# nrclaudio/spVIPES

Measured on AMD Instinct MI355X. Metric: cells/sec/training-step (2-group PoE VAE), higher is better.
Workload: dtype bf16

## Files before the change

include/spvipes_hip.h:

```cpp
#ifndef SPVIPES_HIP_H
#define SPVIPES_HIP_H

#include <stdint.h>

#ifdef __cplusplus
extern "C" {
#endif

#define SPV_OK 0
#define SPV_ERR_ARG (-1)
#define SPV_ERR_LAUNCH (-2)
#define SPV_ERR_UNSUPPORTED (-3)

#define SPV_COUNT_F32 0
#define SPV_COUNT_U16 1

#define SPV_NB_CMAX 64
#define SPV_DEC_KP 16
#define SPV_DEC_KS 32
#define SPV_DEC_KP_WIDE 32
#define SPV_DEC_KS_WIDE 64
#define SPV_DEC_CELLS_PER_WG 128

int spv_version(void);
// ... 109 lines not shown
int spv_dec_heads_wgrad(const uint16_t* tP, const uint16_t* tS, int32_t a_tiles, const uint16_t* Aps, int32_t G, int32_t Bp,
                        int32_t splits, float* slabP, float* slabS, void* stream);

int spv_dec_logits(const uint16_t* Am_hi, const uint16_t* Am_lo, const uint16_t* Wm_hi, const uint16_t* Wm_lo,
                   int32_t K, int32_t Bp, int32_t Gp, int32_t nsplit, void* out, int32_t out_f32, void* stream);

typedef struct spv_dec_params {
  const void* X; int64_t ldx; const int32_t* rows; int32_t col_off; int32_t count_is_u16;
  int32_t B, G, Bp, Gp;
  const void* logits; int32_t n_gene_tiles; int32_t logits_f32;
  const uint16_t* Wps_hi; const uint16_t* Wps_lo;
  const uint16_t* Aps_hi; const uint16_t* Aps_lo;
  const void* gene_tab;
  const void* cnt_tab;
  const float* a_p; const float* a_s; const float* lse_p; const float* lse_s;
  const float* w_row;
  int32_t gene_splits; int32_t genes_per_split;
  float* part_max_p; float* part_sum_p; float* part_max_s; float* part_sum_s;
  float* rec_part; float* tp_part; float* ts_part;
  float* dtheta_part;
  void* dL; void* tP; void* tS; int32_t grads_f32;
  int32_t nb_splits; int32_t nb_genes_per_split;
  int32_t nb_cell_tiles;
  int32_t kslots;
} spv_dec_params;

int spv_dec_tables(const float* px_r, int32_t G, int32_t Gp, void* gene_tab, void* cnt_tab, void* stream);

int spv_dec_lse(const spv_dec_params* p, const float* library, void* stream);

int spv_dec_nb_fwd(const spv_dec_params* p, int32_t train, void* stream);

typedef struct spv_dec_group {
  spv_dec_params p;
  const float* library;
  const float* px_r;
  const uint16_t* Am_hi; const uint16_t* Am_lo; const uint16_t* Wm_hi; const uint16_t* Wm_lo; int32_t K, nsplit;
  const float* Tp; const float* Ts; float* dz_part; float* dw_part;
} spv_dec_group;
int spv_dec_tables_grouped(const spv_dec_group* groups, int32_t n_groups, void* stream);
int spv_dec_logits_grouped(const spv_dec_group* groups, int32_t n_groups, void* stream);
int spv_dec_lse_grouped(const spv_dec_group* groups, int32_t n_groups, void* stream);
int spv_dec_nb_fwd_grouped(const spv_dec_group* groups, int32_t n_groups, int32_t train, void* stream);
int spv_dec_heads_bwd_grouped(const spv_dec_group* groups, int32_t n_groups, void* stream);

int spv_dec_materialize(const spv_dec_params* p, float* scale_private, float* scale_shared, float* rate_private, float* rate_shared,
// ... 259 lines not shown
```

spvipes_amd/_abi.py:

```python
from __future__ import annotations

import ctypes as C
import os
from typing import NamedTuple, Optional

import torch

_HERE = os.path.dirname(os.path.abspath(__file__))
LIB_PATH = os.path.join(_HERE, "_lib", "libspvipes_hip.so")

SPV_COUNT_F32, SPV_COUNT_U16 = 0, 1
NB_CMAX, DEC_KP, DEC_KS, DEC_CELLS_PER_WG = 64, 16, 32, 128
DEC_KPS = DEC_KP + DEC_KS


class DecSlots(NamedTuple):
    kslots: int
    KP: int
    KS: int
    KPS: int


DEC_NARROW = DecSlots(0, DEC_KP, DEC_KS, DEC_KPS)
DEC_WIDE = DecSlots(1, 32, 64, 96)


class SpvCounts(C.Structure):
    _fields_ = [("X", C.c_void_p), ("ld", C.c_int64), ("rows", C.c_void_p), ("col_off", C.c_int32), ("dtype", C.c_int32)]


class SpvDecParams(C.Structure):
    _fields_ = [
        ("X", C.c_void_p), ("ldx", C.c_int64), ("rows", C.c_void_p), ("col_off", C.c_int32), ("count_is_u16", C.c_int32),
        ("B", C.c_int32), ("G", C.c_int32), ("Bp", C.c_int32), ("Gp", C.c_int32),
        ("logits", C.c_void_p), ("n_gene_tiles", C.c_int32), ("logits_f32", C.c_int32),
        ("Wps_hi", C.c_void_p), ("Wps_lo", C.c_void_p), ("Aps_hi", C.c_void_p), ("Aps_lo", C.c_void_p),
        ("gene_tab", C.c_void_p), ("cnt_tab", C.c_void_p),
        ("a_p", C.c_void_p), ("a_s", C.c_void_p), ("lse_p", C.c_void_p), ("lse_s", C.c_void_p), ("w_row", C.c_void_p),
        ("gene_splits", C.c_int32), ("genes_per_split", C.c_int32),
        ("part_max_p", C.c_void_p), ("part_sum_p", C.c_void_p), ("part_max_s", C.c_void_p), ("part_sum_s", C.c_void_p),
        ("rec_part", C.c_void_p), ("tp_part", C.c_void_p), ("ts_part", C.c_void_p), ("dtheta_part", C.c_void_p),
        ("dL", C.c_void_p), ("tP", C.c_void_p), ("tS", C.c_void_p), ("grads_f32", C.c_int32),
        ("nb_splits", C.c_int32), ("nb_genes_per_split", C.c_int32), ("nb_cell_tiles", C.c_int32),
        ("kslots", C.c_int32),
    ]


class SpvReduceProb(C.Structure):
    _fields_ = [("src", C.c_void_p), ("slab_stride", C.c_int64), ("ld_src", C.c_int64), ("nslabs", C.c_int32), ("col_off", C.c_int32),
                ("rows", C.c_int32), ("cols", C.c_int32), ("dst", C.c_void_p), ("ld_dst", C.c_int64), ("accumulate", C.c_int32),
                ("pad_", C.c_int32), ("alpha", C.c_void_p), ("exp_scale", C.c_void_p)]


SPV_MAXR = 16


class SpvReduceBatch(C.Structure):
    _fields_ = [("p", SpvReduceProb * SPV_MAXR), ("nprob", C.c_int32)]


SPV_MAXP = 8
POE_LMAX = 1024
BN_ROWS = 32


class SpvLinearProb(C.Structure):
# ... 346 lines not shown
```

spvipes_amd/csrc/spv_abi.hip:

```cpp
#include "../../include/spvipes_hip.h"
#include "spv_common.h"
#include "spv_gemm.h"
#include "spv_fc1.h"
#include "spv_dec_gemm.h"
#include "spv_decoder.h"
#include "spv_dec_expected.h"
#include "spv_de.h"
#include "spv_de_median.h"
#include "spv_small.h"
#include "spv_poe_n.h"

#include <cstdio>
#include <cstdlib>
#include <cstring>

using namespace spv;

static thread_local char g_err[512] = "";
static int fail(int code, const char* fmt, const char* what = "") {
  snprintf(g_err, sizeof(g_err), fmt, what);
  return code;
}
static int launch_status(const char* what) {
  hipError_t e = hipGetLastError();
// ... 456 lines not shown
    return fail(SPV_ERR_ARG, "spv_dec_heads_wgrad: operands must be 16-byte aligned%s");
  static bool raised = false;
  if (!raised) { (void)hipFuncSetAttribute(reinterpret_cast<const void*>(dec_heads_wgrad_dma_kernel), hipFuncAttributeMaxDynamicSharedMemorySize, DH_LDS_BYTES); raised = true; }
  const int mtiles = (G + DH_BM - 1) / DH_BM, ktiles = Bp / DH_BK;
  const int k_per_split = (ktiles + splits - 1) / splits * DH_BK;
  hipLaunchKernelGGL(dec_heads_wgrad_dma_kernel, dim3(mtiles * splits), dim3(512), DH_LDS_BYTES, (hipStream_t)stream, (const bf16_t*)tP, (const bf16_t*)tS, a_tiles,
                     (const bf16_t*)Aps, G, Bp, k_per_split, splits, slabP, slabS);
  return launch_status("spv_dec_heads_wgrad");
}

static int to_dec(const spv_dec_params* q, DecParams& p) {
  if (!q) return fail(SPV_ERR_ARG, "decoder: null params%s");
  p.X = q->X; p.ldx = q->ldx; p.rows = q->rows; p.col_off = q->col_off; p.count_is_u16 = q->count_is_u16;
  p.B = q->B; p.G = q->G; p.Bp = q->Bp; p.Gp = q->Gp;
  p.logits = q->logits; p.n_gene_tiles = q->n_gene_tiles; p.logits_f32 = q->logits_f32;
  p.Wps_hi = q->Wps_hi; p.Wps_lo = q->Wps_lo; p.Aps_hi = q->Aps_hi; p.Aps_lo = q->Aps_lo;
  p.gene_tab = (const float4*)q->gene_tab; p.cnt_tab = (const float2*)q->cnt_tab;
  p.a_p = q->a_p; p.a_s = q->a_s; p.lse_p = q->lse_p; p.lse_s = q->lse_s; p.w_row = q->w_row;
  p.gene_splits = q->gene_splits; p.genes_per_split = q->genes_per_split;
  p.part_max_p = q->part_max_p; p.part_sum_p = q->part_sum_p; p.part_max_s = q->part_max_s; p.part_sum_s = q->part_sum_s;
  p.rec_part = q->rec_part; p.tp_part = q->tp_part; p.ts_part = q->ts_part; p.dtheta_part = q->dtheta_part;
  p.dL = q->dL; p.tP = q->tP; p.tS = q->tS; p.grads_f32 = q->grads_f32;
  p.nb_splits = q->nb_splits; p.nb_genes_per_split = q->nb_genes_per_split; p.nb_cell_tiles = q->nb_cell_tiles > 0 ? q->nb_cell_tiles : 1;
  if (p.B <= 0 || p.G <= 0 || p.Bp < p.B || p.Gp < p.G || (p.Bp % DEC_CELLS_PER_WG) || (p.Gp % 32))
    return fail(SPV_ERR_ARG, "decoder: Bp must be a multiple of 128 and Gp of 32%s");
  if ((long)p.Bp * p.Gp * (p.grads_f32 ? 2 : 1) >= (1L << 30) || p.Gp >= (1 << 24))
    return fail(SPV_ERR_ARG, "decoder: Bp * Gp must stay below 2^30 elements (and Gp below 2^24)%s");
  if (p.gene_splits <= 0 || (p.genes_per_split % 32) || (long)p.gene_splits * p.genes_per_split < p.G)
    return fail(SPV_ERR_ARG, "decoder: gene splits must be multiples of 32 covering G%s");
  if (!p.Wps_hi || !p.Wps_lo || !p.Aps_hi || !p.Aps_lo) return fail(SPV_ERR_ARG, "decoder: missing packed regressor operands%s");
  if (q->kslots != 0 && q->kslots != 1) return fail(SPV_ERR_ARG, "decoder: kslots must be 0 (16 / 32 K slots) or 1 (32 / 64)%s");
  return SPV_OK;
}
static inline int dec_kw(const spv_dec_params* q) { return q->kslots ? 2 : 1; }

extern "C" int spv_dec_tables(const float* px_r, int32_t G, int32_t Gp, void* gene_tab, void* cnt_tab, void* stream) {
  if (!px_r || !gene_tab || !cnt_tab || G <= 0 || Gp < G) return fail(SPV_ERR_ARG, "spv_dec_tables: bad arguments%s");
  hipLaunchKernelGGL(nb_tables_kernel, dim3((Gp + 255) / 256, NB_CMAX), dim3(256), 0, (hipStream_t)stream, px_r, G, Gp,
                     (float4*)gene_tab, (float2*)cnt_tab);
  return launch_status("spv_dec_tables");
}

extern "C" int spv_dec_tables_grouped(const spv_dec_group* g, int32_t n, void* stream) {
  if (!g || n <= 0) return fail(SPV_ERR_ARG, "spv_dec_tables_grouped: bad arguments%s");
  int i = 0;
  for (; i + 1 < n; i += 2) {
// ... 37 lines not shown
  int i = 0;
  for (; i + 1 < n; i += 2) {
    DecParams p0, p1;
    int rc = lse_prepare(&g[i].p, g[i].library, p0);
    if (rc != SPV_OK) return rc;
    rc = lse_prepare(&g[i + 1].p, g[i + 1].library, p1);
    if (rc != SPV_OK) return rc;
    if (dec_kw(&g[i].p) != dec_kw(&g[i + 1].p)) break;
    const int bp = p0.Bp > p1.Bp ? p0.Bp : p1.Bp, gs = p0.gene_splits > p1.gene_splits ? p0.gene_splits : p1.gene_splits;
    if (dec_kw(&g[i].p) == 2) hipLaunchKernelGGL(dec_lse_pair_kernel<2>, dim3(bp / DEC_CELLS_PER_WG, gs, 2), dim3(256), 0, s, p0, p1);
    else hipLaunchKernelGGL(dec_lse_pair_kernel<1>, dim3(bp / DEC_CELLS_PER_WG, gs, 2), dim3(256), 0, s, p0, p1);
    const LseCombArgs c0{p0.part_max_p, p0.part_sum_p, p0.part_max_s, p0.part_sum_s, p0.gene_splits, p0.Bp, p0.B, g[i].library, (float*)p0.lse_p, (float*)p0.lse_s, (float*)p0.a_p, (float*)p0.a_s};
    const LseCombArgs c1{p1.part_max_p, p1.part_sum_p, p1.part_max_s, p1.part_sum_s, p1.gene_splits, p1.Bp, p1.B, g[i + 1].library, (float*)p1.lse_p, (float*)p1.lse_s, (float*)p1.a_p, (float*)p1.a_s};
    hipLaunchKernelGGL(dec_lse_combine_pair_kernel, dim3((bp + 63) / 64, 1, 2), dim3(256), 0, s, c0, c1);
    if (hipGetLastError() != hipSuccess) return launch_status("spv_dec_lse_grouped");
  }
  for (; i < n; ++i) {
    const int rc = spv_dec_lse(&g[i].p, g[i].library, stream);
    if (rc != SPV_OK) return rc;
  }
  return SPV_OK;
}

template <bool TRAIN, typename GT, int CM, int KW>
static void nb_launch_mode(const DecParams& p, hipStream_t s) {
  const int ctiles = (p.Bp + NB_CELLS_PER_WG - 1) / NB_CELLS_PER_WG;
  dim3 grid((ctiles + p.nb_cell_tiles - 1) / p.nb_cell_tiles, p.nb_splits);
  if (p.logits_f32) hipLaunchKernelGGL((dec_nb_kernel<TRAIN, GT, float, CM, KW>), grid, dim3(256), 0, s, p);
  else hipLaunchKernelGGL((dec_nb_kernel<TRAIN, GT, _Float16, CM, KW>), grid, dim3(256), 0, s, p);
}
template <bool TRAIN, typename GT, int KW>
static void nb_launch_kw(const DecParams& p, hipStream_t s) {
  if (!p.count_is_u16) return nb_launch_mode<TRAIN, GT, CNT_F32, KW>(p, s);
  const bool aligned = ((reinterpret_cast<uintptr_t>(p.X) & 7) == 0) && (p.ldx % 4 == 0) && (p.col_off % 4 == 0);
  if (aligned) nb_launch_mode<TRAIN, GT, CNT_U16_ALIGNED, KW>(p, s);
  else nb_launch_mode<TRAIN, GT, CNT_U16_ANY, KW>(p, s);
}
template <bool TRAIN, typename GT>
static void nb_launch(const DecParams& p, int kw, hipStream_t s) {
  if (kw == 2) nb_launch_kw<TRAIN, GT, 2>(p, s);
  else nb_launch_kw<TRAIN, GT, 1>(p, s);
}

static int nb_prepare(const spv_dec_params* q, int32_t train, DecParams& p) {
  int rc = to_dec(q, p);
  if (rc != SPV_OK) return rc;
  if (!p.X || !p.logits || !p.gene_tab || !p.cnt_tab || !p.a_p || !p.a_s || !p.w_row || !p.rec_part)
    return fail(SPV_ERR_ARG, "spv_dec_nb_fwd: null pointer%s");
  if (p.n_gene_tiles != p.Gp / 32) return fail(SPV_ERR_ARG, "spv_dec_nb_fwd: n_gene_tiles must be Gp / 32%s");
  if (p.nb_splits <= 0 || p.nb_genes_per_split <= 0 || (p.nb_genes_per_split % 32) || p.nb_genes_per_split > NB_GSPL_MAX ||
      (long)p.nb_splits * p.nb_genes_per_split < p.G)
    return fail(SPV_ERR_ARG, "spv_dec_nb_fwd: nb_genes_per_split must be a multiple of 32, at most 160, and the splits must cover G%s");
  if (train && (!p.dL || !p.tP || !p.tS || !p.tp_part || !p.ts_part || !p.dtheta_part))
    return fail(SPV_ERR_ARG, "spv_dec_nb_fwd: training outputs missing%s");
  return SPV_OK;
}
extern "C" int spv_dec_nb_fwd(const spv_dec_params* q, int32_t train, void* stream) {
  DecParams p;
  int rc = nb_prepare(q, train, p);
  if (rc != SPV_OK) return rc;
  hipStream_t s = (hipStream_t)stream;
  const int kw = dec_kw(q);
  if (train) {
    if (p.grads_f32) nb_launch<true, split_t>(p, kw, s);
    else nb_launch<true, bf16_t>(p, kw, s);
  } else {
    nb_launch<false, bf16_t>(p, kw, s);
  }
  return launch_status("spv_dec_nb_fwd");
}
static int nb_count_mode(const DecParams& p) {
// ... 9 lines not shown
  else hipLaunchKernelGGL((dec_nb_pair_kernel<TRAIN, GT, _Float16, CM, KW>), grid, dim3(256), 0, s, p0, p1);
}
template <bool TRAIN, typename GT, int KW>
static void nb_launch_pair_kw(const DecParams& p0, const DecParams& p1, int cm, hipStream_t s) {
  if (cm == CNT_F32) nb_launch_pair_mode<TRAIN, GT, CNT_F32, KW>(p0, p1, s);
  else if (cm == CNT_U16_ALIGNED) nb_launch_pair_mode<TRAIN, GT, CNT_U16_ALIGNED, KW>(p0, p1, s);
  else nb_launch_pair_mode<TRAIN, GT, CNT_U16_ANY, KW>(p0, p1, s);
}
template <bool TRAIN, typename GT>
static void nb_launch_pair(const DecParams& p0, const DecParams& p1, int cm, int kw, hipStream_t s) {
  if (kw == 2) nb_launch_pair_kw<TRAIN, GT, 2>(p0, p1, cm, s);
  else nb_launch_pair_kw<TRAIN, GT, 1>(p0, p1, cm, s);
}
extern "C" int spv_dec_nb_fwd_grouped(const spv_dec_group* g, int32_t n, int32_t train, void* stream) {
  if (!g || n <= 0) return fail(SPV_ERR_ARG, "spv_dec_nb_fwd_grouped: bad arguments%s");
  hipStream_t s = (hipStream_t)stream;
  int i = 0;
  for (; i + 1 < n; i += 2) {
    DecParams p0, p1;
    int rc = nb_prepare(&g[i].p, train, p0);
    if (rc != SPV_OK) return rc;
    rc = nb_prepare(&g[i + 1].p, train, p1);
    if (rc != SPV_OK) return rc;
    if (nb_count_mode(p0) != nb_count_mode(p1) || p0.logits_f32 != p1.logits_f32 || p0.grads_f32 != p1.grads_f32 || dec_kw(&g[i].p) != dec_kw(&g[i + 1].p)) break;
    const int cm = nb_count_mode(p0), kw = dec_kw(&g[i].p);
    if (train) {
      if (p0.grads_f32) nb_launch_pair<true, split_t>(p0, p1, cm, kw, s);
      else nb_launch_pair<true, bf16_t>(p0, p1, cm, kw, s);
    } else {
      nb_launch_pair<false, bf16_t>(p0, p1, cm, kw, s);
    }
    if (hipGetLastError() != hipSuccess) return launch_status("spv_dec_nb_fwd_grouped");
  }
  for (; i < n; ++i) {
    const int rc = spv_dec_nb_fwd(&g[i].p, train, stream);
    if (rc != SPV_OK) return rc;
  }
  return SPV_OK;
}

extern "C" int spv_dec_logits(const uint16_t* Am_hi, const uint16_t* Am_lo, const uint16_t* Wm_hi, const uint16_t* Wm_lo,
                              int32_t K, int32_t Bp, int32_t Gp, int32_t nsplit, void* out, int32_t out_f32, void* stream) {
  if (!Am_hi || !Wm_hi || !out) return fail(SPV_ERR_ARG, "spv_dec_logits: null pointer%s");
  if (K <= 0 || (K % 32) || Bp <= 0 || Gp <= 0 || (Bp % 128) || (Gp % 128)) return fail(SPV_ERR_ARG, "spv_dec_logits: bad shape%s");
  if (nsplit != 1 && nsplit != 3) return fail(SPV_ERR_ARG, "spv_dec_logits: nsplit must be 1 or 3%s");
  if (nsplit == 3 && (!Am_lo || !Wm_lo)) return fail(SPV_ERR_ARG, "spv_dec_logits: nsplit=3 needs lo images%s");
// ... 1385 lines not shown
```

spvipes_amd/csrc/spv_decoder.h:

```cpp
#pragma once
#include "spv_common.h"

namespace spv {

constexpr int NB_CMAX = 64;
constexpr int DEC_KP = 16;
constexpr int DEC_KS = 32;
constexpr int DEC_KPS = DEC_KP + DEC_KS;
template <int KW> constexpr int DEC_KP_W = 16 * KW;
template <int KW> constexpr int DEC_KS_W = 32 * KW;
template <int KW> constexpr int DEC_KPS_W = 48 * KW;
constexpr int DEC_CELLS_PER_WG = 128;

struct DecParams {
  const void* X; long ldx; const int* rows; int col_off; int count_is_u16;
  int B, G;
  int Bp, Gp;
  const void* logits; int n_gene_tiles; int logits_f32;
  const bf16_t* Wps_hi; const bf16_t* Wps_lo;
  const bf16_t* Aps_hi; const bf16_t* Aps_lo;
  const float4* gene_tab;
  const float2* cnt_tab;
  const float* a_p; const float* a_s;
  const float* lse_p; const float* lse_s;
  const float* w_row;
  int gene_splits; int genes_per_split;
  float* part_max_p; float* part_sum_p; float* part_max_s; float* part_sum_s;
  float* rec_part; float* tp_part; float* ts_part;
  float* dtheta_part;
  void* dL; void* tP; void* tS; int grads_f32;
  int nb_splits; int nb_genes_per_split;
  int nb_cell_tiles;
};

__device__ __forceinline__ void nb_tables_body(const float* px_r, int G, int Gp, float4* gene_tab, float2* cnt_tab) {
  const int g = blockIdx.x * blockDim.x + threadIdx.x;
  const int c = blockIdx.y;
  if (g >= Gp) return;
  if (g >= G) {
    if (c == 0) gene_tab[g] = make_float4(1.f, 0.f, 1.f, 0.f);
    cnt_tab[(long)c * Gp + g] = make_float2(0.f, 0.f);
    return;
  }
  const float theta = fast_exp(px_r[g]);
  if (c == 0) {
    const float lt = fast_log(theta + SPV_EPS_NB);
    gene_tab[g] = make_float4(theta, lt, fmaf(theta, fast_rcp(theta + SPV_EPS_NB), lt), theta * lt * 1.4426950408889634f);
    cnt_tab[g] = make_float2(0.f, 0.f);
    return;
  }
  const float x = log1p_count((float)c);
  const LgammaDigamma t = lgamma_digamma(theta), xt = lgamma_digamma(x + theta), x1 = lgamma_digamma(x + 1.0f);
  cnt_tab[(long)c * Gp + g] = make_float2(xt.lg - t.lg - x1.lg, xt.dg - t.dg);
}
__global__ void nb_tables_kernel(const float* px_r, int G, int Gp, float4* gene_tab, float2* cnt_tab) { nb_tables_body(px_r, G, Gp, gene_tab, cnt_tab); }
// ... 294 lines not shown

typedef __attribute__((ext_vector_type(4))) float f4acc;
constexpr float NB_LN2 = 0.6931471805599453f, NB_LOG2E = 1.4426950408889634f;
constexpr int NB_GSPL_MAX = 160;
constexpr int NB_WPITCH = 56;
constexpr int NB_CELLS_PER_WG = 64;

#ifndef SPV_NB_ABLATE
#define SPV_NB_ABLATE 0
#endif
#ifdef SPV_NB_STAMPS
__device__ unsigned long long* g_nb_stamps;
#define NB_STAMP(i) do { if (threadIdx.x == 0) { unsigned long long t_; asm volatile("s_memtime %0\n\ts_waitcnt lgkmcnt(0)" : "=s"(t_) :: "memory"); g_nb_stamps[((size_t)blockIdx.y * gridDim.x + blockIdx.x) * 8 + (i)] = t_; } } while (0)
#else
#define NB_STAMP(i) do { } while (0)
#endif
#ifndef SPV_NB_OCC
#define SPV_NB_OCC 3
#endif
constexpr int NB_WPITCH_WIDE = 104;
constexpr int SPV_NB_OCC_WIDE = 2;
template <int KW> constexpr int NB_WPITCH_W = KW == 1 ? NB_WPITCH : NB_WPITCH_WIDE;
template <int KW> constexpr int NB_OCC_W = KW == 1 ? SPV_NB_OCC : SPV_NB_OCC_WIDE;
template <bool TRAIN, typename GT, typename LT, int CM, int KW = 1>
__device__ __forceinline__ void dec_nb_body(const DecParams& p) {
  constexpr int DEC_KP = DEC_KP_W<KW>, DEC_KPS = DEC_KPS_W<KW>, NB_WPITCH = NB_WPITCH_W<KW>;
  constexpr int NSK = DEC_KS_W<KW> / 32;
  __shared__ __attribute__((aligned(16))) bf16_t s_whi[NB_GSPL_MAX * NB_WPITCH], s_wlo[NB_GSPL_MAX * NB_WPITCH];
  __shared__ float4 s_gt[NB_GSPL_MAX];
  __shared__ float s_dth[TRAIN ? 4 : 1][NB_GSPL_MAX];
  const int tid = threadIdx.x, lane = tid & 63, wave = tid >> 6;
  const int c16 = lane & 15, gq = lane >> 4;
  const int split = blockIdx.y;
  const int gbeg = split * p.nb_genes_per_split;
  int gend = gbeg + p.nb_genes_per_split;
  if (gend > p.Gp) gend = p.Gp;
  if (gend > ((p.G + 15) & ~15)) gend = (p.G + 15) & ~15;
  const int ng = gend - gbeg;
  NB_STAMP(0);
  const int nct = p.nb_cell_tiles;
  if (ng <= 0) {
    for (int ct = 0; ct < nct; ++ct) {
      const int cell = (blockIdx.x * nct + ct) * NB_CELLS_PER_WG + tid;
      if (cell < p.Bp) {
        const long o = (long)split * p.Bp + cell;
        p.rec_part[o] = 0.f;
        if constexpr (TRAIN) { p.tp_part[o] = 0.f; p.ts_part[o] = 0.f; }
      }
    }
    return;
  }
  for (int i = tid; i < ng * (DEC_KPS / 8); i += 256) {
    const int row = i / (DEC_KPS / 8), ch = i % (DEC_KPS / 8);
    *reinterpret_cast<u4v*>(s_whi + row * NB_WPITCH + 8 * ch) = *reinterpret_cast<const u4v*>(p.Wps_hi + (long)(gbeg + row) * DEC_KPS + 8 * ch);
    *reinterpret_cast<u4v*>(s_wlo + row * NB_WPITCH + 8 * ch) = *reinterpret_cast<const u4v*>(p.Wps_lo + (long)(gbeg + row) * DEC_KPS + 8 * ch);
  }
  for (int i = tid; i < ng; i += 256) s_gt[i] = p.gene_tab[gbeg + i];
  __syncthreads();
  NB_STAMP(1);
  const int nchunks = ng >> 4;

  for (int ct = 0; ct < nct; ++ct) {
    const int tile16 = (blockIdx.x * nct + ct) * (NB_CELLS_PER_WG / 16) + wave;
    if (tile16 * 16 >= p.Bp) break;
    const int cell = tile16 * 16 + c16;
    const int cell_tile = tile16 >> 1, chh = tile16 & 1;
    const bool cell_ok = cell < p.B;
    const long aoff = (long)cell * DEC_KPS + 8 * gq;
    s8v bp_hi = *reinterpret_cast<const s8v*>(p.Aps_hi + aoff), bp_lo = *reinterpret_cast<const s8v*>(p.Aps_lo + aoff);
    if (DEC_KP == 16 && gq >= 2) {
#pragma unroll
      for (int i = 0; i < 8; ++i) { bp_hi[i] = 0; bp_lo[i] = 0; }
    }
    s8v bs_hi[NSK], bs_lo[NSK];
#pragma unroll
    for (int s = 0; s < NSK; ++s) {
      bs_hi[s] = *reinterpret_cast<const s8v*>(p.Aps_hi + aoff + DEC_KP + 32 * s);
      bs_lo[s] = *reinterpret_cast<const s8v*>(p.Aps_lo + aoff + DEC_KP + 32 * s);
    }
    const float ap2 = p.a_p[cell] * NB_LOG2E, as2 = p.a_s[cell] * NB_LOG2E;
    const float w = p.w_row[cell];
    const long row_of_cell = ((SPV_NB_ABLATE & 16) != 0) ? 0 : (cell_ok ? (p.rows ? (long)p.rows[cell] : (long)cell) : 0);
    float rec = 0.f, tp_sum = 0.f, ts_sum = 0.f;
    const int lane_st = (16 * chh + c16 + 32 * (gq & 1)) * 4 + (gq >> 1) * 256;
    const unsigned tile_row = (unsigned)cell_tile * (unsigned)p.n_gene_tiles;
    const unsigned plane = (unsigned)p.Bp * (unsigned)p.Gp;
    auto tile_off = [&](int g0) { return (tile_row + (unsigned)(g0 >> 5)) * 1024u + (unsigned)(((g0 >> 4) & 1) * 512 + lane_st); };
    auto gather_tab = [&](const float (&c)[4], int g0, float2 (&tab)[4]) {
#pragma unroll
      for (int j = 0; j < 4; ++j) {
        unsigned eo = __umul24((unsigned)(int)__builtin_amdgcn_fmed3f(c[j], 0.f, (float)(NB_CMAX - 1)), (unsigned)p.Gp) + (unsigned)(g0 + 4 * gq + j);
        if constexpr ((SPV_NB_ABLATE & 2) != 0) eo = (unsigned)(g0 + 4 * gq + j);
        tab[j] = *reinterpret_cast<const float2*>(reinterpret_cast<const char*>(p.cnt_tab) + (size_t)(eo * 8u));
      }
    };

    RawCounts<CM> rawA = load_counts4_raw<CM>(p, row_of_cell, gbeg + 4 * gq, cell_ok), rawB = rawA, rawC = rawA;
    float ellA[4];
    float2 tabA[4];
    load4b<LT>(p.logits, tile_off(gbeg), ellA);
    if (nchunks > 1) rawB = load_counts4_raw<CM>(p, row_of_cell, gbeg + 16 + 4 * gq, cell_ok);
    {
      float c0[4];
      decode_counts4<CM>(p, rawA, row_of_cell, gbeg + 4 * gq, cell_ok, c0);
      gather_tab(c0, gbeg, tabA);
    }

    NB_STAMP(2);
    for (int c = 0; c < nchunks; ++c) {
      if (c == 1) NB_STAMP(3);
      const int g0 = gbeg + 16 * c;
      const unsigned toff = tile_off(g0);
      const int wrow = (16 * c + c16) * NB_WPITCH + 8 * gq;
      const s8v wp_hi = *reinterpret_cast<const s8v*>(s_whi + wrow), wp_lo = *reinterpret_cast<const s8v*>(s_wlo + wrow);
      f4acc yp = {0.f, 0.f, 0.f, 0.f}, ys = {0.f, 0.f, 0.f, 0.f};
      yp = __builtin_amdgcn_mfma_f32_16x16x32_bf16(wp_hi, bp_lo, yp, 0, 0, 0);
      yp = __builtin_amdgcn_mfma_f32_16x16x32_bf16(wp_lo, bp_hi, yp, 0, 0, 0);
      yp = __builtin_amdgcn_mfma_f32_16x16x32_bf16(wp_hi, bp_hi, yp, 0, 0, 0);
#pragma unroll
      for (int s = 0; s < NSK; ++s) {
        const s8v ws_hi = *reinterpret_cast<const s8v*>(s_whi + wrow + DEC_KP + 32 * s), ws_lo = *reinterpret_cast<const s8v*>(s_wlo + wrow + DEC_KP + 32 * s);
        ys = __builtin_amdgcn_mfma_f32_16x16x32_bf16(ws_hi, bs_lo[s], ys, 0, 0, 0);
        ys = __builtin_amdgcn_mfma_f32_16x16x32_bf16(ws_lo, bs_hi[s], ys, 0, 0, 0);
        ys = __builtin_amdgcn_mfma_f32_16x16x32_bf16(ws_hi, bs_hi[s], ys, 0, 0, 0);
      }
      const int g1 = gbeg + 16 * min(c + 1, nchunks - 1), g2 = gbeg + 16 * min(c + 2, nchunks - 1);
      float ellB[4];
      float2 tabB[4];
      rawC = load_counts4_raw<CM>(p, row_of_cell, g2 + 4 * gq, cell_ok);
      if constexpr ((SPV_NB_ABLATE & 4) != 0) { ellB[0] = ellA[1]; ellB[1] = ellA[2]; ellB[2] = ellA[3]; ellB[3] = ellA[0]; }
      else load4b<LT>(p.logits, tile_off(g1), ellB);
      {
        float cB[4];
        decode_counts4<CM>(p, rawB, row_of_cell, g1 + 4 * gq, cell_ok, cB);
        gather_tab(cB, g1, tabB);
      }
      float cntA[4];
      decode_counts4<CM>(p, rawA, row_of_cell, g0 + 4 * gq, cell_ok, cntA);
      const int gq0 = g0 + 4 * gq;
      float o_dl[4], o_tp[4], o_ts[4], dth4[4];
#pragma unroll
      for (int j = 0; j < 4; ++j) {
        const int g = gq0 + j;
        const bool ok = cell_ok && (g < p.G);
        const float4 gt = s_gt[g - gbeg];
        const float theta = gt.x, dlt = gt.z, thlt2 = gt.w;
        const float cj = cntA[j];
        const float x = log1p_count(cj);
        const float F = tabA[j].x, Psi = tabA[j].y;
        const float el_ = ellA[j];
        const float mu1 = __builtin_amdgcn_exp2f(fmaf(yp[j], NB_LOG2E, ap2)), mu2 = __builtin_amdgcn_exp2f(fmaf(ys[j], NB_LOG2E, as2));
        const float e1 = mu1 + SPV_EPS_NB, e2 = mu2 + SPV_EPS_NB;
        const float S1 = theta + e1, S2 = theta + e2;
// ... 51 lines not shown
        } else {
        store_grad4<GT>(p.dL, toff, plane, o_dl);
        store_grad4<GT>(p.tP, toff, plane, o_tp);
        store_grad4<GT>(p.tS, toff, plane, o_ts);
        }
        if constexpr ((SPV_NB_ABLATE & 8) != 0) { asm volatile("" ::"v"(dth4[0]), "v"(dth4[1]), "v"(dth4[2]), "v"(dth4[3])); } else {
        const bool u3 = lane & 8, u2 = lane & 4;
        const float a0 = (u3 ? dth4[2] : dth4[0]) + __shfl_xor(u3 ? dth4[0] : dth4[2], 8, 64);
        const float a1 = (u3 ? dth4[3] : dth4[1]) + __shfl_xor(u3 ? dth4[1] : dth4[3], 8, 64);
        float s = (u2 ? a1 : a0) + __shfl_xor(u2 ? a0 : a1, 4, 64);
        s += __shfl_xor(s, 2, 64);
        s += __shfl_xor(s, 1, 64);
        if ((lane & 3) == 0) {
          float* slot = &s_dth[wave][16 * c + 4 * gq + 2 * ((lane >> 3) & 1) + ((lane >> 2) & 1)];
          *slot = (ct == 0) ? s : *slot + s;
        }
        }
      }

#pragma unroll
      for (int j = 0; j < 4; ++j) { ellA[j] = ellB[j]; tabA[j] = tabB[j]; }
      rawA = rawB; rawB = rawC;
    }
    NB_STAMP(4);
    rec += __shfl_xor(rec, 16, 64); rec += __shfl_xor(rec, 32, 64);
    if constexpr (TRAIN) {
      tp_sum += __shfl_xor(tp_sum, 16, 64); tp_sum += __shfl_xor(tp_sum, 32, 64);
      ts_sum += __shfl_xor(ts_sum, 16, 64); ts_sum += __shfl_xor(ts_sum, 32, 64);
    }
    if (gq == 0) {
      const long o = (long)split * p.Bp + cell;
      p.rec_part[o] = rec;
      if constexpr (TRAIN) { p.tp_part[o] = tp_sum; p.ts_part[o] = ts_sum; }
    }
  }
  if constexpr (TRAIN) {
    __syncthreads();
    for (int i = tid; i < ng; i += 256)
      p.dtheta_part[(long)blockIdx.x * p.Gp + gbeg + i] = ((s_dth[0][i] + s_dth[1][i]) + s_dth[2][i]) + s_dth[3][i];
  }
  NB_STAMP(5);
}
template <bool TRAIN, typename GT, typename LT, int CM, int KW = 1>
__global__ __launch_bounds__(256, NB_OCC_W<KW>) void dec_nb_kernel(DecParams p) { dec_nb_body<TRAIN, GT, LT, CM, KW>(p); }
template <bool TRAIN, typename GT, typename LT, int CM, int KW = 1>
__global__ __launch_bounds__(256, NB_OCC_W<KW>) void dec_nb_pair_kernel(DecParams p0, DecParams p1) {
  const DecParams p = blockIdx.z ? p1 : p0;
  const int ctiles = (p.Bp + NB_CELLS_PER_WG - 1) / NB_CELLS_PER_WG;
  if ((int)blockIdx.x >= (ctiles + p.nb_cell_tiles - 1) / p.nb_cell_tiles || (int)blockIdx.y >= p.nb_splits) return;
  dec_nb_body<TRAIN, GT, LT, CM, KW>(p);
}

template <typename LT, int KW = 1>
__global__ __launch_bounds__(256) void dec_materialize_kernel(DecParams p, float* scale_p, float* scale_s, float* rate_p, float* rate_s,
                                                              float* logits_out, long ld) {
  const int lane = threadIdx.x & 63, wave = threadIdx.x >> 6, h = lane >> 5, r = lane & 31;
  const int cell_tile = blockIdx.x * (DEC_CELLS_PER_WG / 32) + wave;
  const int cell0 = cell_tile * 32, cell = cell0 + r;
  PsFragsK<KW> cf;
  load_ps_cell_frags(p, cell0, lane, cf);
  const float lp = p.lse_p[cell], ls = p.lse_s[cell], ap = p.a_p[cell], as = p.a_s[cell];
  const int gbeg = blockIdx.y * p.genes_per_split;
  int gend = gbeg + p.genes_per_split;
  if (gend > p.Gp) gend = p.Gp;
  if (gend > ((p.G + 31) & ~31)) gend = (p.G + 31) & ~31;
  for (int g0 = gbeg; g0 < gend; g0 += 32) {
    PsWK<KW> w;
// ... 666 lines not shown
```

spvipes_amd/dec_ops.py:

```python
from __future__ import annotations

import ctypes as C
from typing import List, Optional, Sequence

import numpy as np
import torch

from . import _abi
from ._abi import (DEC_CELLS_PER_WG, DEC_NARROW, NB_CMAX, TRUNK_KMAX, SpvBnBatch, SpvDecExpectedArgs, SpvDecGroup, SpvDecParams, SpvFoldBatch, SpvGemmArgs, SpvReduceBatch, SpvTrunkBatch, SpvZsplitArgs,
                   ptr, round_up, stream_ptr)
from .nn_ops import _add_lin, _fptr, _lin_batch, _wgrad, grad_out
from . import ops as _ops
from .ops import N_HIDDEN_MIX, GroupCounts, Workspace, _bf16_image, _gemm_slabs, _gene_splits, _nb_cell_tiles, _nb_splits, _pack, fork, group_streams, join

N_DEC_PARAMS = 13
KMP = 320


def dec_slots(decoder):
    return getattr(decoder, "dec_slots", DEC_NARROW)


def _slab_cols(KP: int, KS: int):
    return [(0, KP, 0, 0)] + [(KP + c, 32, 1, c) for c in range(0, KS, 32)]
# ... 291 lines not shown
            raise _abi.SpvError("DecoderFused: w_pad must be contiguous fp32 of length >= round_up(B, 128)")
        grads_f32 = bool(need_grad and mlo)
        gdt, gname, gplanes = (torch.int16, "split", 2) if grads_f32 else (torch.int16, "bf16", 1)
        P, saved_g = [], []
        rec = [new(B) for _ in range(NG)]
        red = SpvReduceBatch()
        red.nprob = 0
        if _ops.OVERLAP_SMALL:
            torch.cuda.current_stream(dev).wait_stream(side)
        streams = group_streams(dev, NG) if (_ops.FWD_GROUP_STREAMS and not pair) else [torch.cuda.current_stream(dev)] * NG
        fork(streams)
        dgrp = (SpvDecGroup * NG)() if pair else None
        lib_keep = []
        for g in range(NG):
          with torch.cuda.stream(streams[g]):
              G, Gp, wsg = Gs[g], Gps[g], ws[g]
              (Wm_hi, Wm_lo), (gene_tab, cnt_tab) = Wm_img[g], tabs[g]
              (Am_hi, Am_lo), (Aps_hi, Aps_lo) = Am_img[g], Aps_img[g]
              if not fused_pack:
                  _pack(m[g], Am_hi, Am_lo, dst_col_off=0, cslot=n_m)
                  _pack(zcat[g], Am_hi, Am_lo, extra_one=True, dst_col_off=n_m, cslot=KMP - n_m)
                  _pack(zcat[g][:, :n_p], Aps_hi, Aps_lo, extra_one=True, dst_col_off=0, cslot=DEC_KP)
                  _pack(zcat[g][:, n_p:], Aps_hi, Aps_lo, extra_one=True, dst_col_off=DEC_KP, cslot=DEC_KS)
              logits = wsg.get("dec_logits_" + ("f32" if mlo else "f16"), (Bp, Gp), torch.float32 if mlo else torch.float16)
              lse_first = bool(_ops.STAGGER and g % 2 == 1)
              if not lse_first and not pair:
                  _abi.call("spv_dec_logits", ptr(Am_hi), ptr(Am_lo), ptr(Wm_hi), ptr(Wm_lo), KMP, Bp, Gp, nsplit, ptr(logits), int(mlo), stream_ptr())
              splits, per = _gene_splits(Bp, Gp)
              nbs, nbper = _nb_splits(Gp, Bp)
              vec = lambda nme: wsg.get(nme, (Bp,), torch.float32)
              part = lambda nme: wsg.get(nme, (splits, Bp), torch.float32)
              nbpart = lambda nme: wsg.get(nme, (nbs, Bp), torch.float32)
              if need_grad:
                  dL = wsg.get("dec_dL_" + gname, (gplanes * Bp, Gp), gdt, zero=True)
                  tP = wsg.get("dec_tP_" + gname, (gplanes * Bp, Gp), gdt, zero=True)
                  tS = wsg.get("dec_tS_" + gname, (gplanes * Bp, Gp), gdt, zero=True)
                  dth = wsg.get("dec_dtheta", (Bp // 64, Gp), torch.float32, zero=True)
                  Tp, Ts = wsg.get("dec_Tp", (Bp,), torch.float32), wsg.get("dec_Ts", (Bp,), torch.float32)
              else:
                  dL = tP = tS = dth = Tp = Ts = None
              lse_p, lse_s, a_p, a_s = vec("dec_lse_p"), vec("dec_lse_s"), vec("dec_a_p"), vec("dec_a_s")
              cst = counts[g].c_struct(rows[g])
              p = SpvDecParams(
                  X=cst.X, ldx=cst.ld, rows=cst.rows, col_off=cst.col_off, count_is_u16=int(cst.dtype == _abi.SPV_COUNT_U16),
                  B=B, G=G, Bp=Bp, Gp=Gp, logits=ptr(logits), n_gene_tiles=Gp // 32, logits_f32=int(mlo),
                  Wps_hi=ptr(Wps[g][0]), Wps_lo=ptr(Wps[g][1]), Aps_hi=ptr(Aps_hi), Aps_lo=ptr(Aps_lo),
                  gene_tab=ptr(gene_tab), cnt_tab=ptr(cnt_tab), a_p=ptr(a_p), a_s=ptr(a_s), lse_p=ptr(lse_p), lse_s=ptr(lse_s),
                  w_row=ptr(w_pad), gene_splits=splits, genes_per_split=per,
                  part_max_p=ptr(part("dec_pmp")), part_sum_p=ptr(part("dec_psp")), part_max_s=ptr(part("dec_pms")), part_sum_s=ptr(part("dec_pss")),
                  rec_part=ptr(nbpart("dec_rec")), tp_part=ptr(nbpart("dec_tp")), ts_part=ptr(nbpart("dec_ts")),
                  dtheta_part=ptr(dth), dL=ptr(dL), tP=ptr(tP), tS=ptr(tS), grads_f32=int(grads_f32), nb_splits=nbs, nb_genes_per_split=nbper,
                  nb_cell_tiles=_nb_cell_tiles(Bp, Gp), kslots=sl.kslots,
              )
              if pair:
                  lib_keep.append(cont(library[g].flatten()))
                  q = dgrp[g]
                  q.p, q.library = p, ptr(lib_keep[-1])
                  q.Am_hi, q.Am_lo, q.Wm_hi, q.Wm_lo, q.K, q.nsplit = ptr(Am_hi), ptr(Am_lo), ptr(Wm_hi), ptr(Wm_lo), KMP, nsplit
              else:
                  _abi.call("spv_dec_lse", C.byref(p), ptr(cont(library[g].flatten())), stream_ptr())
                  if lse_first:
                      _abi.call("spv_dec_logits", ptr(Am_hi), ptr(Am_lo), ptr(Wm_hi), ptr(Wm_lo), KMP, Bp, Gp, nsplit, ptr(logits), int(mlo), stream_ptr())
                  _abi.call("spv_dec_nb_fwd", C.byref(p), int(need_grad), stream_ptr())
              r = rec[g]
              _add_red(red, nbpart("dec_rec"), nbs, Bp, Bp, 1, B, r, B)
              if need_grad:
                  _add_red(red, nbpart("dec_tp"), nbs, Bp, Bp, 1, Bp, Tp, Bp)
                  _add_red(red, nbpart("dec_ts"), nbs, Bp, Bp, 1, Bp, Ts, Bp)
              P.append(p)
              if need_grad:
                  saved_g.append(dict(Wm=(Wm_hi, Wm_lo), Am=(Am_hi, Am_lo), Aps=(Aps_hi, Aps_lo), dL=dL, tP=tP, tS=tS, dth=dth, Tp=Tp, Ts=Ts))
        join(streams)
        if pair:
            _abi.call("spv_dec_logits_grouped", dgrp, NG, stream_ptr())
            _abi.call("spv_dec_lse_grouped", dgrp, NG, stream_ptr())
            _abi.call("spv_dec_nb_fwd_grouped", dgrp, NG, int(need_grad), stream_ptr())
        _run_red(red)
        loss, rec_sum, gkl = new(()), new(()), new(B)
        klp = (C.c_void_p * 4)(*[ptr(k) for k in kls], *([None] * (4 - n_kl)))
        _abi.call("spv_loss_assemble", ptr(rec[0]), ptr(rec[1]) if NG > 1 else None, ptr(w_pad), klp, n_kl, B, ptr(klw), ptr(loss), ptr(rec_sum), ptr(gkl), stream_ptr())
        if need_grad:
            ctx.P, ctx.saved_g, ctx.ws, ctx.decoders, ctx.training, ctx.nsplit = P, saved_g, ws, decoders, training, nsplit
            ctx.dims = (B, Bp, Gs, Gps, n_p, n_s, n_m, KM)
            ctx.NG = NG
# ... 416 lines not shown
```

spvipes_amd/ops.py:

```python
from __future__ import annotations

import ctypes as C
import os
from dataclasses import dataclass
from typing import Dict, Optional, Tuple

import torch

from . import _abi
from ._abi import DEC_CELLS_PER_WG, NB_CMAX, SpvCounts, SpvDecParams, check, ptr, round_up, stream_ptr

N_HIDDEN_MIX = 256


@dataclass
class GroupCounts:

    X: torch.Tensor
    G: int
    col_off: int = 0
    resident: bool = False

    def __post_init__(self):
        self._xb = None
# ... 243 lines not shown
DEC_PAIR = os.environ.get("SPV_DEC_PAIR", "auto")


def dec_pair_for(B: int, n_groups: int) -> bool:
    if n_groups != 2 or DEC_PAIR == "0":
        return False
    return True if DEC_PAIR == "1" else _SMALL_STEP


FC1_PAIR_SPLITS = os.environ.get("SPV_FC1_PAIR_SPLITS", "1") != "0"
DEC_PAIR_SPLITS = os.environ.get("SPV_DEC_PAIR_SPLITS", "1") != "0"
HEADS_DMA = os.environ.get("SPV_HEADS_DMA", "1") != "0"
FUSED_HEADS = os.environ.get("SPV_FUSED_HEADS", "1") != "0"
GSPLIT_WANT = int(os.environ.get("SPV_GSPLIT_WANT", "512"))
FUSED_HEADS_F32 = os.environ.get("SPV_FUSED_HEADS_F32", "1") != "0"
FUSED_DZ = os.environ.get("SPV_FUSED_DZ", "1") != "0"
FUSED_DZ_F32 = os.environ.get("SPV_FUSED_DZ_F32", "1") != "0"
DA_FIXUP = os.environ.get("SPV_DA_FIXUP", "0")
TRUNK_FOLD = os.environ.get("SPV_TRUNK_FOLD", "1") != "0"
FUSED_PACK = os.environ.get("SPV_FUSED_PACK", "1") != "0"
DEFER_WM = os.environ.get("SPV_DEFER_WM", "1") != "0"
DEFER_BC = os.environ.get("SPV_DEFER_BC", "1") != "0"
DZ_ONLY = os.environ.get("SPV_DZ_ONLY", "0") != "0"
FWD_GROUP_STREAMS = os.environ.get("SPV_FWD_GROUP_STREAMS", "1") != "0"
BWD_GROUP_STREAMS = os.environ.get("SPV_BWD_GROUP_STREAMS", "1") != "0"
_PENDING: list = []
_PENDING_KEEP: list = []


def defer(stream, keep=()) -> None:
    if stream not in _PENDING:
        _PENDING.append(stream)
    _PENDING_KEEP.extend(keep)


def join_all_side_streams(device) -> None:
    dev = torch.device(device)
    cur = torch.cuda.current_stream(dev)
    capturing = torch.cuda.is_current_stream_capturing()
    for (idx, _i), st in _SIDE_STREAMS.items():
        if idx != dev.index or st is cur:
            continue
        if capturing:
            with torch.cuda.stream(st):
                if not torch.cuda.is_current_stream_capturing():
                    continue
# ... 271 lines not shown
```

Measured before the change: 6.125 million.

## Fuse decoder logits GEMM into the NB likelihood kernel with LDS-pipelined weights

Adds a fused-logits variant of the NB forward kernel. It computes each 16-gene logit chunk in-kernel with bf16 MFMA, streaming Wm chunks into a triple-buffered, swizzled LDS ring via global_load_lds DMA. This removes the separate logits GEMM launch and the Bp×Gp f16 logits write and re-read. The path runs only for non-pair, narrow-slot, f16-logit, bf16-grad configurations. It lowers occupancy to 2 and computes logits from the hi bf16 words only, which may change numerics.

```diff
diff --git a/include/spvipes_hip.h b/include/spvipes_hip.h
--- a/include/spvipes_hip.h
+++ b/include/spvipes_hip.h
@@ -155,6 +155,7 @@
   void* dL; void* tP; void* tS; int32_t grads_f32;
   int32_t nb_splits; int32_t nb_genes_per_split;
   int32_t nb_cell_tiles;
+  const uint16_t* Wm; const uint16_t* Am; int32_t KM;
   int32_t kslots;
 } spv_dec_params;
 
diff --git a/spvipes_amd/_abi.py b/spvipes_amd/_abi.py
--- a/spvipes_amd/_abi.py
+++ b/spvipes_amd/_abi.py
@@ -42,6 +42,7 @@
         ("rec_part", C.c_void_p), ("tp_part", C.c_void_p), ("ts_part", C.c_void_p), ("dtheta_part", C.c_void_p),
         ("dL", C.c_void_p), ("tP", C.c_void_p), ("tS", C.c_void_p), ("grads_f32", C.c_int32),
         ("nb_splits", C.c_int32), ("nb_genes_per_split", C.c_int32), ("nb_cell_tiles", C.c_int32),
+        ("Wm", C.c_void_p), ("Am", C.c_void_p), ("KM", C.c_int32),
         ("kslots", C.c_int32),
     ]
 
diff --git a/spvipes_amd/csrc/spv_abi.hip b/spvipes_amd/csrc/spv_abi.hip
--- a/spvipes_amd/csrc/spv_abi.hip
+++ b/spvipes_amd/csrc/spv_abi.hip
@@ -502,6 +502,7 @@
   p.rec_part = q->rec_part; p.tp_part = q->tp_part; p.ts_part = q->ts_part; p.dtheta_part = q->dtheta_part;
   p.dL = q->dL; p.tP = q->tP; p.tS = q->tS; p.grads_f32 = q->grads_f32;
   p.nb_splits = q->nb_splits; p.nb_genes_per_split = q->nb_genes_per_split; p.nb_cell_tiles = q->nb_cell_tiles > 0 ? q->nb_cell_tiles : 1;
+  p.Wm = (const bf16_t*)q->Wm; p.Am = (const bf16_t*)q->Am; p.KM = q->KM;
   if (p.B <= 0 || p.G <= 0 || p.Bp < p.B || p.Gp < p.G || (p.Bp % DEC_CELLS_PER_WG) || (p.Gp % 32))
     return fail(SPV_ERR_ARG, "decoder: Bp must be a multiple of 128 and Gp of 32%s");
   if ((long)p.Bp * p.Gp * (p.grads_f32 ? 2 : 1) >= (1L << 30) || p.Gp >= (1 << 24))
@@ -585,10 +586,19 @@
   return SPV_OK;
 }
 
+static bool nb_fused_logits(const DecParams& p, int kw) {
+  return p.Wm && p.Am && !p.grads_f32 && !p.logits_f32 && kw == 1 && p.nb_cell_tiles == 1 && (p.Bp % NB_CELLS_PER_WG) == 0;
+}
 template <bool TRAIN, typename GT, int CM, int KW>
 static void nb_launch_mode(const DecParams& p, hipStream_t s) {
   const int ctiles = (p.Bp + NB_CELLS_PER_WG - 1) / NB_CELLS_PER_WG;
   dim3 grid((ctiles + p.nb_cell_tiles - 1) / p.nb_cell_tiles, p.nb_splits);
+  if constexpr (KW == 1 && sizeof(GT) == 2) {
+    if (nb_fused_logits(p, KW)) {
+      hipLaunchKernelGGL((dec_nb_kernel<TRAIN, bf16_t, _Float16, CM, 1, true>), grid, dim3(256), 0, s, p);
+      return;
+    }
+  }
   if (p.logits_f32) hipLaunchKernelGGL((dec_nb_kernel<TRAIN, GT, float, CM, KW>), grid, dim3(256), 0, s, p);
   else hipLaunchKernelGGL((dec_nb_kernel<TRAIN, GT, _Float16, CM, KW>), grid, dim3(256), 0, s, p);
 }
@@ -608,8 +618,13 @@
 static int nb_prepare(const spv_dec_params* q, int32_t train, DecParams& p) {
   int rc = to_dec(q, p);
   if (rc != SPV_OK) return rc;
-  if (!p.X || !p.logits || !p.gene_tab || !p.cnt_tab || !p.a_p || !p.a_s || !p.w_row || !p.rec_part)
+  if (!p.X || !p.gene_tab || !p.cnt_tab || !p.a_p || !p.a_s || !p.w_row || !p.rec_part)
     return fail(SPV_ERR_ARG, "spv_dec_nb_fwd: null pointer%s");
+  if ((p.Wm != nullptr) != (p.Am != nullptr)) return fail(SPV_ERR_ARG, "spv_dec_nb_fwd: Wm and Am come together%s");
+  if (p.Wm && (p.KM <= 0 || (p.KM % 32) || p.KM > NB_FL_K || ((reinterpret_cast<uintptr_t>(p.Wm) | reinterpret_cast<uintptr_t>(p.Am)) & 15)))
+    return fail(SPV_ERR_ARG, "spv_dec_nb_fwd: Wm / Am must be 16-byte aligned [.][320] images and KM a multiple of 32, at most 320%s");
+  if (!p.logits && !nb_fused_logits(p, dec_kw(q)))
+    return fail(SPV_ERR_ARG, "spv_dec_nb_fwd: logits missing (the fused-logits kernel takes bf16 gradient words, f16 logits, kslots 0 and nb_cell_tiles 1)%s");
   if (p.n_gene_tiles != p.Gp / 32) return fail(SPV_ERR_ARG, "spv_dec_nb_fwd: n_gene_tiles must be Gp / 32%s");
   if (p.nb_splits <= 0 || p.nb_genes_per_split <= 0 || (p.nb_genes_per_split % 32) || p.nb_genes_per_split > NB_GSPL_MAX ||
       (long)p.nb_splits * p.nb_genes_per_split < p.G)
@@ -665,6 +680,7 @@
     if (rc != SPV_OK) return rc;
     rc = nb_prepare(&g[i + 1].p, train, p1);
     if (rc != SPV_OK) return rc;
+    if (!p0.logits || !p1.logits) return fail(SPV_ERR_ARG, "spv_dec_nb_fwd_grouped: the pair grid reads precomputed logits%s");
     if (nb_count_mode(p0) != nb_count_mode(p1) || p0.logits_f32 != p1.logits_f32 || p0.grads_f32 != p1.grads_f32 || dec_kw(&g[i].p) != dec_kw(&g[i + 1].p)) break;
     const int cm = nb_count_mode(p0), kw = dec_kw(&g[i].p);
     if (train) {
diff --git a/spvipes_amd/csrc/spv_decoder.h b/spvipes_amd/csrc/spv_decoder.h
--- a/spvipes_amd/csrc/spv_decoder.h
+++ b/spvipes_amd/csrc/spv_decoder.h
@@ -1,5 +1,6 @@
 #pragma once
 #include "spv_common.h"
+#include "spv_fc1.h"
 
 namespace spv {
 
@@ -31,6 +32,8 @@
   void* dL; void* tP; void* tS; int grads_f32;
   int nb_splits; int nb_genes_per_split;
   int nb_cell_tiles;
+  const bf16_t* Wm; const bf16_t* Am;
+  int KM;
 };
 
 __device__ __forceinline__ void nb_tables_body(const float* px_r, int G, int Gp, float4* gene_tab, float2* cnt_tab) {
@@ -371,10 +374,21 @@
 constexpr int SPV_NB_OCC_WIDE = 2;
 template <int KW> constexpr int NB_WPITCH_W = KW == 1 ? NB_WPITCH : NB_WPITCH_WIDE;
 template <int KW> constexpr int NB_OCC_W = KW == 1 ? SPV_NB_OCC : SPV_NB_OCC_WIDE;
-template <bool TRAIN, typename GT, typename LT, int CM, int KW = 1>
+__device__ __forceinline__ void nb_dma16(const unsigned char* src, unsigned lds_base) {
+  asm volatile("s_mov_b32 m0, %1\n\ts_nop 0\n\tglobal_load_lds_dwordx4 %0, off" ::"v"(src), "s"(lds_base) : "memory", "m0");
+}
+constexpr int NB_FL_K = 320;
+constexpr int NB_FL_STEPS = NB_FL_K / 32;
+constexpr int NB_FL_CHUNK_ELEMS = 16 * NB_FL_K;
+constexpr int NB_FL_NBUF = 3;
+constexpr int NB_FL_PIECES = NB_FL_CHUNK_ELEMS * 2 / 1024;
+constexpr int NB_FL_ISSUES = 3;
+template <bool TRAIN, typename GT, typename LT, int CM, int KW = 1, bool FL = false>
 __device__ __forceinline__ void dec_nb_body(const DecParams& p) {
   constexpr int DEC_KP = DEC_KP_W<KW>, DEC_KPS = DEC_KPS_W<KW>, NB_WPITCH = NB_WPITCH_W<KW>;
   constexpr int NSK = DEC_KS_W<KW> / 32;
+  static_assert(!FL || (KW == 1 && sizeof(GT) == 2 && sizeof(LT) == 2), "fused logits: bf16 gradient words, f16-logits mode, narrow layout");
+  __shared__ __attribute__((aligned(16))) bf16_t s_wm[FL ? NB_FL_NBUF * NB_FL_CHUNK_ELEMS : 8];
   __shared__ __attribute__((aligned(16))) bf16_t s_whi[NB_GSPL_MAX * NB_WPITCH], s_wlo[NB_GSPL_MAX * NB_WPITCH];
   __shared__ float4 s_gt[NB_GSPL_MAX];
   __shared__ float s_dth[TRAIN ? 4 : 1][NB_GSPL_MAX];
@@ -408,10 +422,33 @@
   __syncthreads();
   NB_STAMP(1);
   const int nchunks = ng >> 4;
+  unsigned wm_src[NB_FL_ISSUES];
+  int wm_dst[NB_FL_ISSUES];
+  if constexpr (FL) {
+    const int wv = uniform_wave_id();
+#pragma unroll
+    for (int i = 0; i < NB_FL_ISSUES; ++i) {
+      const int piece = min(wv + 4 * i, NB_FL_PIECES - 1);
+      const int u = 64 * piece + lane, row = u / (NB_FL_K / 8), pos = u % (NB_FL_K / 8);
+      wm_src[i] = (unsigned)((row * NB_FL_K + 8 * (pos ^ ((row >> 1) & 7))) * 2);
+      wm_dst[i] = piece * 1024;
+    }
+  }
+  auto wm_issue = [&](int src_chunk, int slot) {
+    const unsigned char* src = reinterpret_cast<const unsigned char*>(p.Wm) + (long)(gbeg + 16 * src_chunk) * (NB_FL_K * 2);
+    const unsigned dst = lds_addr_of(reinterpret_cast<const unsigned char*>(s_wm)) + (unsigned)(slot * (NB_FL_CHUNK_ELEMS * 2));
+#pragma unroll
+    for (int i = 0; i < NB_FL_ISSUES; ++i) nb_dma16(src + wm_src[i], __builtin_amdgcn_readfirstlane(dst + wm_dst[i]));
+  };
+  constexpr int NB_FL_YOUNGER = NB_FL_ISSUES + 1 + 4 + (TRAIN ? 3 : 0);
 
   for (int ct = 0; ct < nct; ++ct) {
     const int tile16 = (blockIdx.x * nct + ct) * (NB_CELLS_PER_WG / 16) + wave;
     if (tile16 * 16 >= p.Bp) break;
+    if constexpr (FL) {
+      if (ct > 0) lds_barrier();
+      wm_issue(0, 0);
+    }
     const int cell = tile16 * 16 + c16;
     const int cell_tile = tile16 >> 1, chh = tile16 & 1;
     const bool cell_ok = cell < p.B;
@@ -426,6 +463,11 @@
     for (int s = 0; s < NSK; ++s) {
       bs_hi[s] = *reinterpret_cast<const s8v*>(p.Aps_hi + aoff + DEC_KP + 32 * s);
       bs_lo[s] = *reinterpret_cast<const s8v*>(p.Aps_lo + aoff + DEC_KP + 32 * s);
+    }
+    s8v am[FL ? NB_FL_STEPS : 1];
+    if constexpr (FL) {
+#pragma unroll
+      for (int s = 0; s < NB_FL_STEPS; ++s) am[s] = *reinterpret_cast<const s8v*>(p.Am + (long)cell * NB_FL_K + 32 * s + 8 * gq);
     }
     const float ap2 = p.a_p[cell] * NB_LOG2E, as2 = p.a_s[cell] * NB_LOG2E;
     const float w = p.w_row[cell];
@@ -447,19 +489,39 @@
     RawCounts<CM> rawA = load_counts4_raw<CM>(p, row_of_cell, gbeg + 4 * gq, cell_ok), rawB = rawA, rawC = rawA;
     float ellA[4];
     float2 tabA[4];
-    load4b<LT>(p.logits, tile_off(gbeg), ellA);
+    if constexpr (!FL) load4b<LT>(p.logits, tile_off(gbeg), ellA);
     if (nchunks > 1) rawB = load_counts4_raw<CM>(p, row_of_cell, gbeg + 16 + 4 * gq, cell_ok);
     {
       float c0[4];
       decode_counts4<CM>(p, rawA, row_of_cell, gbeg + 4 * gq, cell_ok, c0);
       gather_tab(c0, gbeg, tabA);
     }
+    if constexpr (FL) {
+      __builtin_amdgcn_sched_barrier(0);
+      wm_issue(min(1, nchunks - 1), 1);
+      asm volatile("s_waitcnt vmcnt(%0)" ::"n"(NB_FL_ISSUES) : "memory");
+    }
 
     NB_STAMP(2);
     for (int c = 0; c < nchunks; ++c) {
       if (c == 1) NB_STAMP(3);
       const int g0 = gbeg + 16 * c;
       const unsigned toff = tile_off(g0);
+      f4acc lg = {0.f, 0.f, 0.f, 0.f};
+      if constexpr (FL) {
+        asm volatile("s_waitcnt vmcnt(%0)" ::"n"(NB_FL_YOUNGER) : "memory");
+        lds_barrier();
+        const bf16_t* const wb = s_wm + (c % NB_FL_NBUF) * NB_FL_CHUNK_ELEMS + c16 * NB_FL_K;
+        const int sw = (c16 >> 1) & 7;
+        s8v wmf[NB_FL_STEPS];
+#pragma unroll
+        for (int s = 0; s < NB_FL_STEPS; ++s) wmf[s] = *reinterpret_cast<const s8v*>(wb + 8 * ((4 * s + gq) ^ sw));
+        __builtin_amdgcn_sched_barrier(0);
+        wm_issue(min(c + 2, nchunks - 1), (c + 2) % NB_FL_NBUF);
+        __builtin_amdgcn_sched_barrier(0);
+#pragma unroll
+        for (int s = 0; s < NB_FL_STEPS; ++s) lg = __builtin_amdgcn_mfma_f32_16x16x32_bf16(wmf[s], am[s], lg, 0, 0, 0);
+      }
       const int wrow = (16 * c + c16) * NB_WPITCH + 8 * gq;
       const s8v wp_hi = *reinterpret_cast<const s8v*>(s_whi + wrow), wp_lo = *reinterpret_cast<const s8v*>(s_wlo + wrow);
       f4acc yp = {0.f, 0.f, 0.f, 0.f}, ys = {0.f, 0.f, 0.f, 0.f};
@@ -477,7 +539,10 @@
       float ellB[4];
       float2 tabB[4];
       rawC = load_counts4_raw<CM>(p, row_of_cell, g2 + 4 * gq, cell_ok);
-      if constexpr ((SPV_NB_ABLATE & 4) != 0) { ellB[0] = ellA[1]; ellB[1] = ellA[2]; ellB[2] = ellA[3]; ellB[3] = ellA[0]; }
+      if constexpr (FL) {
+#pragma unroll
+        for (int j = 0; j < 4; ++j) { ellA[j] = (float)(_Float16)lg[j]; ellB[j] = 0.f; }
+      } else if constexpr ((SPV_NB_ABLATE & 4) != 0) { ellB[0] = ellA[1]; ellB[1] = ellA[2]; ellB[2] = ellA[3]; ellB[3] = ellA[0]; }
       else load4b<LT>(p.logits, tile_off(g1), ellB);
       {
         float cB[4];
@@ -575,6 +640,7 @@
       for (int j = 0; j < 4; ++j) { ellA[j] = ellB[j]; tabA[j] = tabB[j]; }
       rawA = rawB; rawB = rawC;
     }
+    if constexpr (FL) asm volatile("s_waitcnt vmcnt(0)" ::: "memory");
     NB_STAMP(4);
     rec += __shfl_xor(rec, 16, 64); rec += __shfl_xor(rec, 32, 64);
     if constexpr (TRAIN) {
@@ -594,8 +660,8 @@
   }
   NB_STAMP(5);
 }
-template <bool TRAIN, typename GT, typename LT, int CM, int KW = 1>
-__global__ __launch_bounds__(256, NB_OCC_W<KW>) void dec_nb_kernel(DecParams p) { dec_nb_body<TRAIN, GT, LT, CM, KW>(p); }
+template <bool TRAIN, typename GT, typename LT, int CM, int KW = 1, bool FL = false>
+__global__ __launch_bounds__(256, FL ? 2 : NB_OCC_W<KW>) void dec_nb_kernel(DecParams p) { dec_nb_body<TRAIN, GT, LT, CM, KW, FL>(p); }
 template <bool TRAIN, typename GT, typename LT, int CM, int KW = 1>
 __global__ __launch_bounds__(256, NB_OCC_W<KW>) void dec_nb_pair_kernel(DecParams p0, DecParams p1) {
   const DecParams p = blockIdx.z ? p1 : p0;
diff --git a/spvipes_amd/dec_ops.py b/spvipes_amd/dec_ops.py
--- a/spvipes_amd/dec_ops.py
+++ b/spvipes_amd/dec_ops.py
@@ -337,9 +337,10 @@
                   _pack(zcat[g], Am_hi, Am_lo, extra_one=True, dst_col_off=n_m, cslot=KMP - n_m)
                   _pack(zcat[g][:, :n_p], Aps_hi, Aps_lo, extra_one=True, dst_col_off=0, cslot=DEC_KP)
                   _pack(zcat[g][:, n_p:], Aps_hi, Aps_lo, extra_one=True, dst_col_off=DEC_KP, cslot=DEC_KS)
-              logits = wsg.get("dec_logits_" + ("f32" if mlo else "f16"), (Bp, Gp), torch.float32 if mlo else torch.float16)
+              fuse_logits = bool(_ops.NB_FUSE_LOGITS and not pair and not mlo and sl.kslots == 0)
+              logits = None if fuse_logits else wsg.get("dec_logits_" + ("f32" if mlo else "f16"), (Bp, Gp), torch.float32 if mlo else torch.float16)
               lse_first = bool(_ops.STAGGER and g % 2 == 1)
-              if not lse_first and not pair:
+              if not lse_first and not pair and not fuse_logits:
                   _abi.call("spv_dec_logits", ptr(Am_hi), ptr(Am_lo), ptr(Wm_hi), ptr(Wm_lo), KMP, Bp, Gp, nsplit, ptr(logits), int(mlo), stream_ptr())
               splits, per = _gene_splits(Bp, Gp)
               nbs, nbper = _nb_splits(Gp, Bp)
@@ -366,6 +367,7 @@
                   rec_part=ptr(nbpart("dec_rec")), tp_part=ptr(nbpart("dec_tp")), ts_part=ptr(nbpart("dec_ts")),
                   dtheta_part=ptr(dth), dL=ptr(dL), tP=ptr(tP), tS=ptr(tS), grads_f32=int(grads_f32), nb_splits=nbs, nb_genes_per_split=nbper,
                   nb_cell_tiles=_nb_cell_tiles(Bp, Gp), kslots=sl.kslots,
+                  Wm=ptr(Wm_hi) if fuse_logits else None, Am=ptr(Am_hi) if fuse_logits else None, KM=round_up(KM, 32) if fuse_logits else 0,
               )
               if pair:
                   lib_keep.append(cont(library[g].flatten()))
@@ -374,7 +376,7 @@
                   q.Am_hi, q.Am_lo, q.Wm_hi, q.Wm_lo, q.K, q.nsplit = ptr(Am_hi), ptr(Am_lo), ptr(Wm_hi), ptr(Wm_lo), KMP, nsplit
               else:
                   _abi.call("spv_dec_lse", C.byref(p), ptr(cont(library[g].flatten())), stream_ptr())
-                  if lse_first:
+                  if lse_first and not fuse_logits:
                       _abi.call("spv_dec_logits", ptr(Am_hi), ptr(Am_lo), ptr(Wm_hi), ptr(Wm_lo), KMP, Bp, Gp, nsplit, ptr(logits), int(mlo), stream_ptr())
                   _abi.call("spv_dec_nb_fwd", C.byref(p), int(need_grad), stream_ptr())
               r = rec[g]
diff --git a/spvipes_amd/ops.py b/spvipes_amd/ops.py
--- a/spvipes_amd/ops.py
+++ b/spvipes_amd/ops.py
@@ -289,6 +289,7 @@
 DEFER_WM = os.environ.get("SPV_DEFER_WM", "1") != "0"
 DEFER_BC = os.environ.get("SPV_DEFER_BC", "1") != "0"
 DZ_ONLY = os.environ.get("SPV_DZ_ONLY", "0") != "0"
+NB_FUSE_LOGITS = os.environ.get("SPV_NB_FUSE_LOGITS", "1") != "0"
 FWD_GROUP_STREAMS = os.environ.get("SPV_FWD_GROUP_STREAMS", "1") != "0"
 BWD_GROUP_STREAMS = os.environ.get("SPV_BWD_GROUP_STREAMS", "1") != "0"
 _PENDING: list = []
```

Measured after the change: 5.823 million. 0.951x the previous value.
